# pfnet-research/superpixel-align

Hardware: AMD Instinct MI355X
Metric: images/sec superpixel-align labelling (1024x2048) (higher is better)
Workload: dtype f32 as 2 x f16 planes, f32 accumulate

## Files before the change

### superpixel-align_amd/csrc/spa_common.h

```cpp
#pragma once
#include <hip/hip_runtime.h>
#include <stdint.h>
#include <stdio.h>
#include <string.h>

#include "../../include/spalign.h"

#define SPA_WAVE 64

void spa_set_error(const char *fmt, ...);

#define SPA_HIP(call)                                                                  \
    do {                                                                               \
        hipError_t e_ = (call);                                                        \
        if (e_ != hipSuccess) {                                                        \
            spa_set_error("%s failed: %s (%s:%d)", #call, hipGetErrorString(e_),      \
                          __FILE__, __LINE__);                                         \
            return SPA_ERR_HIP;                                                        \
        }                                                                              \
    } while (0)

#define SPA_ARG(cond)                                                                  \
    do {                                                                               \
        if (!(cond)) {                                                                 \
// ... 61 lines not shown
};

enum {
    PROF_RGB2LAB = 0, PROF_SLIC_ASSIGN, PROF_SLIC_UPDATE, PROF_CONNECT, PROF_STATS,
    PROF_CELL_WEIGHTS, PROF_POOL_MEAN, PROF_POOL_ANCHOR, PROF_KMEANS, PROF_PAINT,
    PROF_DRN_STEM, PROF_DRN_BIAS_ACT, PROF_DRN_CONV, PROF_DRN_CONV32, PROF_DRN_GEMM32, PROF_DRN_GEMM32_N, PROF_WINO_IN, PROF_WINO_OUT, PROF_DRN_GEMM16, PROF_DRN_GEMM16_N, PROF_DRN_CONV16, PROF_DRN_CONV16_128, PROF_DRN_CONV16_256, PROF_DRN_CONV16_1X1, PROF_DRN_CONV16_FRONT, PROF_DRN_CONV_LIGHT, PROF_SLOTS
};

struct spa_ctx {
    int device;
    int n_cu;
    uint32_t *d_status;
    unsigned status_takes;
    void *ws[WS_COUNT];
    size_t ws_bytes[WS_COUNT];
    int prof_on;
    hipEvent_t *prof_ev[PROF_SLOTS];
    int prof_cap[PROF_SLOTS], prof_used[PROF_SLOTS];
    hipStream_t aux[2];
    hipEvent_t ev_fork, ev_join[2];
    int aux_ready;
    int km_attr_done[2];
    int conn_attr_done;
    int conn_claim_ready;
    size_t conn_claim_bytes;
    int upd_wg_per_cu, upd_wg_per_cu8;
    int slic_force_general;
    int zero_line_ready, conv_attr_done, conv32_attr_done, fz_attr_done, gemm16_attr_done, gemm16s_attr_done, nprng_attr_done;
    int rng_seeded;
    int ws_generation;
    int dbg_slic_ldsx;
    int convp_on;
    int convs2_on;
    int convs2_attr_done;
    int rs_key[4], rs_ks[2];
};

#ifdef __HIPCC__
__device__ __forceinline__ unsigned spa_split16_pair(float x0, float x1, float sc, unsigned &l)
{
    unsigned h, lo;
    asm("v_fma_mixlo_f16 %0, %2, %4, 0 op_sel_hi:[0,0,0]\n\t"
        "v_fma_mixhi_f16 %0, %3, %4, 0 op_sel_hi:[0,0,0]\n\t"
        "v_fma_mixlo_f16 %1, %2, %4, -%0 op_sel_hi:[0,0,1]\n\t"
        "v_fma_mixhi_f16 %1, %3, %4, -%0 op_sel:[0,0,1] op_sel_hi:[0,0,1]"
        : "=&v"(h), "=&v"(lo) : "v"(x0), "v"(x1), "v"(sc));
    l = lo;
    return h;
}
#endif

int spa_aux_streams(spa_ctx *ctx);

void spa_prof_mark(spa_ctx *ctx, int slot, int end, hipStream_t s);
struct SpaProfScope {
    spa_ctx *c; int slot; hipStream_t s;
    SpaProfScope(spa_ctx *c_, int slot_, hipStream_t s_) : c(c_), slot(slot_), s(s_) { if (c->prof_on && slot >= 0) spa_prof_mark(c, slot, 0, s); }
    ~SpaProfScope() { if (c->prof_on && slot >= 0) spa_prof_mark(c, slot, 1, s); }
};

int spa_ws_reserve(spa_ctx *ctx, int which, size_t bytes, void **out);
void spa_zero_word(void *word, hipStream_t s);

static inline hipStream_t spa_stream(void *s) { return (hipStream_t)s; }

__device__ __forceinline__ double spa_det_log_pos(double x)
{
    unsigned long long b = (unsigned long long)__double_as_longlong(x);
    int e = (int)((b >> 52) & 0x7ff) - 1023;
    b = (b & 0x000fffffffffffffULL) | 0x3ff0000000000000ULL;
    double m = __longlong_as_double((long long)b);
    if (m > 1.4142135623730951) { m = m * 0.5; e += 1; }
    double s = (m - 1.0) / (m + 1.0);
    double z = s * s;
    double p = 1.0 / 25.0;
    p = p * z + 1.0 / 23.0;
    p = p * z + 1.0 / 21.0;
    p = p * z + 1.0 / 19.0;
    p = p * z + 1.0 / 17.0;
    p = p * z + 1.0 / 15.0;
    p = p * z + 1.0 / 13.0;
    p = p * z + 1.0 / 11.0;
    p = p * z + 1.0 / 9.0;
    p = p * z + 1.0 / 7.0;
    p = p * z + 1.0 / 5.0;
    p = p * z + 1.0 / 3.0;
    p = p * z + 1.0;
    double lnm = 2.0 * s * p;
    double ed = (double)e;
    return ed * 6.93147180369123816490e-01 + (ed * 1.90821492927058770002e-10 + lnm);
}

__device__ __forceinline__ double spa_det_exp(double t)
{
    double kf = floor(t * 1.44269504088896338700e+00 + 0.5);
// ... 27 lines not shown
```

### superpixel-align_amd/csrc/spa_ctx.hip

```cpp
#include <math.h>
#include <stdarg.h>
#include <stdlib.h>

#include "spa_common.h"

static thread_local char g_err[512] = "";

void spa_set_error(const char *fmt, ...)
{
    va_list ap;
    va_start(ap, fmt);
    vsnprintf(g_err, sizeof(g_err), fmt, ap);
    va_end(ap);
}

extern "C" const char *spa_last_error(void) { return g_err; }
extern "C" int spa_version(void) { return 100; }

extern "C" int spa_ctx_create(int device, spa_ctx **out)
{
    SPA_ARG(out != nullptr);
    int n = 0;
    if (hipGetDeviceCount(&n) != hipSuccess || n <= 0) {
        spa_set_error("no HIP device visible: libspalign has no CPU fallback");
        return SPA_ERR_NOGPU;
    }
    if (device < 0) SPA_HIP(hipGetDevice(&device));
    SPA_ARG(device < n);
    SPA_HIP(hipSetDevice(device));
    hipDeviceProp_t prop;
    SPA_HIP(hipGetDeviceProperties(&prop, device));
    if (strncmp(prop.gcnArchName, "gfx950", 6) != 0) {
        spa_set_error("device %d is %s; libspalign is built for gfx950 (MI355X) only", device,
                      prop.gcnArchName);
        return SPA_ERR_NOGPU;
    }
    spa_ctx *ctx = (spa_ctx *)calloc(1, sizeof(spa_ctx));
    ctx->device = device;
    ctx->n_cu = prop.multiProcessorCount;
    if (const char *e = getenv("SPA_SLIC_GENERAL")) ctx->slic_force_general = atoi(e) != 0;
    ctx->convp_on = getenv("SPA_CONVP") ? atoi(getenv("SPA_CONVP")) != 0 : 1;
    ctx->convs2_on = 1;
    SPA_HIP(hipMalloc((void **)&ctx->d_status, 32 * sizeof(uint32_t)));
    SPA_HIP(hipMemset(ctx->d_status, 0, 32 * sizeof(uint32_t)));
    *out = ctx;
    return SPA_OK;
}

extern "C" void spa_ctx_destroy(spa_ctx *ctx)
{
    if (!ctx) return;
    for (int i = 0; i < PROF_SLOTS; ++i) {
        for (int j = 0; j < ctx->prof_cap[i]; ++j) (void)hipEventDestroy(ctx->prof_ev[i][j]);
        free(ctx->prof_ev[i]);
    }
    for (int i = 0; i < WS_COUNT; ++i)
        if (ctx->ws[i]) (void)hipFree(ctx->ws[i]);
    if (ctx->d_status) (void)hipFree(ctx->d_status);
    if (ctx->aux_ready) {
        for (int i = 0; i < 2; ++i) { (void)hipStreamDestroy(ctx->aux[i]); (void)hipEventDestroy(ctx->ev_join[i]); }
        (void)hipEventDestroy(ctx->ev_fork);
    }
    free(ctx);
}

__global__ void k_zero_word(unsigned *w) { *w = 0u; }
void spa_zero_word(void *word, hipStream_t s) { hipLaunchKernelGGL(k_zero_word, dim3(1), dim3(1), 0, s, (unsigned *)word); }

int spa_ws_reserve(spa_ctx *ctx, int which, size_t bytes, void **out)
{
    if (bytes == 0) bytes = 16;
    if (ctx->ws_bytes[which] < bytes) {
        SPA_HIP(hipDeviceSynchronize());
        if (ctx->ws[which]) SPA_HIP(hipFree(ctx->ws[which]));
        ctx->ws[which] = nullptr;
// ... 204 lines not shown
        float4 d;
        if (mode == 1) { d.x = ((const volatile float *)q)[0]; d.y = ((const volatile float *)q)[1]; d.z = ((const volatile float *)q)[2]; d.w = ((const volatile float *)q)[3]; }
        else d = *(const float4 *)q;
        const float ty = (float)(e0.x & 31u) - fy;
        const float dy = (jj & 3) == 3 ? INFINITY : ty * ty;
        const dbg_f32x2 p0 = (dbg_f32x2{dy, dy} + dbg_f32x2{d.x, d.y}) * dbg_f32x2{0.37f, 0.37f} + acc0 * dbg_f32x2{0.001f, 0.001f};
        const dbg_f32x2 p1 = (dbg_f32x2{dy, dy} + dbg_f32x2{d.z, d.w}) * dbg_f32x2{0.37f, 0.37f} + acc1 * dbg_f32x2{0.001f, 0.001f};
        const float dd[4] = {p0.x, p0.y, p1.x, p1.y};
#pragma unroll
        for (int i = 0; i < 4; ++i) {
            const bool take = best[i] > dd[i];
            best[i] = take ? dd[i] : best[i];
            bl[i] = take ? jj : bl[i];
        }
        if (p0.x < 1e30f) acc0 = p0;
        if (p1.x < 1e30f) acc1 = p1;
    }
    float4 r = make_float4(best[0] + (float)bl[0], best[1] + (float)bl[1], best[2] + (float)bl[2], best[3] + (float)bl[3]);
    *(float4 *)(out + ((long long)blockIdx.x * 256 + tid) * 4) = r;
}

extern "C" int spa_debug_lds_probe(spa_ctx *ctx, float *out, int32_t n_wg, int32_t steps, int32_t mode, void *stream)
{
    SPA_ARG(ctx && out && n_wg > 0 && steps > 0 && steps <= 32 && mode >= 0 && mode <= 2);
    hipLaunchKernelGGL(k_debug_lds_probe, dim3((unsigned)n_wg), dim3(256), 0, spa_stream(stream), out, steps, mode, 0.731f);
    SPA_LAUNCH_CHECK();
    return SPA_OK;
}

extern "C" int spa_ws_generation(spa_ctx *ctx) { return ctx ? ctx->ws_generation : -1; }

extern "C" int spa_debug_set(spa_ctx *ctx, int32_t key, int32_t value)
{
    SPA_ARG(ctx && (key == 1 || key == 2 || key == 3) && (value == 0 || value == 1));
    if (key == 1) ctx->convp_on = value;
    else if (key == 3) ctx->convs2_on = value;
    else {
#ifdef SPA_DIAG
        ctx->dbg_slic_ldsx = value;
#else
        SPA_ARG(!"spa_debug_set key 2 (the reproducer variant of k_slic_assign) exists in diagnostic builds only: make EXTRA=-DSPA_DIAG");
#endif
    }
    return SPA_OK;
}

extern "C" int spa_debug_peek(spa_ctx *ctx, int which, size_t offset, size_t bytes, void *host)
{
    if (which == -1) which = WS_DEBUG;
    SPA_ARG(ctx && host && which >= 0 && which < WS_COUNT && offset + bytes <= ctx->ws_bytes[which]);
    SPA_HIP(hipDeviceSynchronize());
    SPA_HIP(hipMemcpy(host, (const char *)ctx->ws[which] + offset, bytes, hipMemcpyDeviceToHost));
    return SPA_OK;
}
```

### superpixel-align_amd/csrc/spa_drn.hip

```cpp
#include "spa_common.h"

__device__ __forceinline__ float bf16_to_f32(unsigned short h) { return __uint_as_float(((unsigned)h) << 16); }
__device__ __forceinline__ unsigned short f32_to_bf16(float f)
{
    unsigned u = __float_as_uint(f);
    if ((u & 0x7fffffffu) > 0x7f800000u) return (unsigned short)((u >> 16) | 0x0040u);
    return (unsigned short)((u + 0x7fffu + ((u >> 16) & 1u)) >> 16);
}

__global__ __launch_bounds__(256) void k_drn_normalise(const float *__restrict__ x, void *__restrict__ out,
                                                       long long npix, int out_bf16, double m0, double m1,
                                                       double m2, double s0, double s1, double s2)
{
    const int b = blockIdx.y;
    const float *src = x + (long long)b * 3 * npix;
    const double mean[3] = {m0, m1, m2}, sd[3] = {s0, s1, s2};
    for (long long p = (long long)blockIdx.x * 256 + threadIdx.x; p < npix; p += (long long)gridDim.x * 256) {
        float v[3];
#pragma unroll
        for (int c = 0; c < 3; ++c) {
            float t = src[c * npix + p] / 255.0f;
            t = (float)((double)t - mean[c]);
            t = (float)((double)t / sd[c]);
            v[c] = t;
        }
        const long long o = ((long long)b * npix + p) * 3;
        if (out_bf16) {
            unsigned short *d = (unsigned short *)out + o;
            d[0] = f32_to_bf16(v[0]); d[1] = f32_to_bf16(v[1]); d[2] = f32_to_bf16(v[2]);
        } else {
            float *d = (float *)out + o;
            d[0] = v[0]; d[1] = v[1]; d[2] = v[2];
        }
    }
}

extern "C" int spa_drn_normalise(spa_ctx *ctx, const float *x, int32_t B, int32_t H, int32_t W, void *out,
                                 int32_t out_dtype, const double *mean3_host, const double *std3_host,
                                 void *stream)
{
    SPA_ARG(ctx && x && out && mean3_host && std3_host && B > 0 && H > 0 && W > 0);
    SPA_ARG(out_dtype == 0 || out_dtype == 1);
    const long long npix = (long long)H * W;
    int gx = (int)((npix + 255) / 256);
    if (gx > 2048) gx = 2048;
    hipLaunchKernelGGL(k_drn_normalise, dim3(gx, B), dim3(256), 0, spa_stream(stream), x, out, npix, out_dtype,
                       mean3_host[0], mean3_host[1], mean3_host[2], std3_host[0], std3_host[1], std3_host[2]);
    SPA_LAUNCH_CHECK();
    return SPA_OK;
}

template <bool POW2>
__global__ __launch_bounds__(256) void k_bias_act_f32(float *__restrict__ y, const float *__restrict__ bias,
                                                      const float *__restrict__ res, unsigned n4, unsigned c4,
                                                      int relu, unsigned *__restrict__ amax = nullptr)
{
    const unsigned stride = gridDim.x * 256u;
    unsigned mx = 0u;
    const float4 *b4 = (const float4 *)bias;
    auto bidx = [&](unsigned i) -> unsigned { return POW2 ? (i & (c4 - 1u)) : (i % c4); };
    auto apply = [&](float4 v, const float4 bb, const float4 r) -> float4 {
        v.x = v.x + bb.x; v.y = v.y + bb.y; v.z = v.z + bb.z; v.w = v.w + bb.w;
        if (res) { v.x = v.x + r.x; v.y = v.y + r.y; v.z = v.z + r.z; v.w = v.w + r.w; }
        if (relu) { v.x = fmaxf(v.x, 0.0f); v.y = fmaxf(v.y, 0.0f); v.z = fmaxf(v.z, 0.0f); v.w = fmaxf(v.w, 0.0f); }
        if (amax)
            mx = max(max(mx, __float_as_uint(v.x) & 0x7fffffffu), max(__float_as_uint(v.y) & 0x7fffffffu,
                     max(__float_as_uint(v.z) & 0x7fffffffu, __float_as_uint(v.w) & 0x7fffffffu)));
        return v;
    };
    unsigned i = blockIdx.x * 256u + threadIdx.x;
    const float4 zero = make_float4(0.0f, 0.0f, 0.0f, 0.0f);
    for (; (unsigned long long)i + 3ull * stride < n4; i += 4u * stride) {
        float4 v[4], r[4];
#pragma unroll
        for (int u = 0; u < 4; ++u) v[u] = ((const float4 *)y)[i + u * stride];
#pragma unroll
        for (int u = 0; u < 4; ++u) r[u] = res ? ((const float4 *)res)[i + u * stride] : zero;
#pragma unroll
        for (int u = 0; u < 4; ++u) ((float4 *)y)[i + u * stride] = apply(v[u], b4[bidx(i + u * stride)], r[u]);
    }
// ... 90 lines not shown
```

### superpixel-align_amd/csrc/spa_stem.hip

```cpp
#include "spa_common.h"

#define ST_TH 16
#define ST_TW 32
#define ST_IH (ST_TH + 8)
#define ST_IW (ST_TW + 8)
#define ST_IPLANE (ST_IH * ST_IW + 8)
#define ST_LH (ST_TH + 2)
#define ST_LW (ST_TW + 2)
#define ST_LP (ST_LH * ST_LW)
#define ST_PS 17
#define ST_K0 148
#define ST_S0 (ST_K0 / 4)
#define ST_S1 (144 / 4)
#define ST_PF 8

typedef float stem_f4 __attribute__((ext_vector_type(4)));

__device__ __forceinline__ unsigned short stem_bf16(float f)
{
    const unsigned u = __float_as_uint(f);
    if ((u & 0x7fffffffu) > 0x7f800000u) return (unsigned short)((u >> 16) | 0x0040u);
    return (unsigned short)((u + 0x7fffu + ((u >> 16) & 1u)) >> 16);
}

// ... 292 lines not shown
            stem_f4 acc = {0.0f, 0.0f, 0.0f, 0.0f};
            const unsigned short *lb = l0_s + (row * ST_LW + col) * SB_L0_PITCH;
#pragma unroll
            for (int s = 0; s < 5; ++s) {
                const stem_bf8 f = *(const stem_bf8 *)(lb + l1off[s]);
                acc = __builtin_amdgcn_mfma_f32_16x16x32_bf16(wa1[s], f, acc, 0, 0, 0);
            }
            const int gy = ty0 + row, gx = tx0 + col;
            if (gy < H && gx < W) {
                uint2 o;
                o.x = (unsigned)stem_bf16_rn(fmaxf(acc[0] + bias1.x, 0.0f)) | ((unsigned)stem_bf16_rn(fmaxf(acc[1] + bias1.y, 0.0f)) << 16);
                o.y = (unsigned)stem_bf16_rn(fmaxf(acc[2] + bias1.z, 0.0f)) | ((unsigned)stem_bf16_rn(fmaxf(acc[3] + bias1.w, 0.0f)) << 16);
                *(uint2 *)(yh + ((((long long)b * H + gy) * W + gx) * 16 + 4 * g)) = o;
            }
        }
        stem_lds_barrier();
    }
}

typedef _Float16 stem_h8 __attribute__((ext_vector_type(8)));
#define SH_PW 48
#define SH_PLANE (ST_IH * SH_PW + 16)
#define SH_COPY (3 * SH_PLANE + 48)
#define SH_L0_PITCH 32
#define SH_IN_S0 4096.0f

__device__ __forceinline__ unsigned short stem_f16_bits(float f)
{
    const _Float16 h = (_Float16)f;
    return __builtin_bit_cast(unsigned short, h);
}
__device__ __forceinline__ float stem_f16_val(unsigned short b) { return (float)__builtin_bit_cast(_Float16, b); }

__global__ __launch_bounds__(256, 2) void k_drn_stem_d_f16x3(const float *__restrict__ xn, int B, int H, int W,
                                                             const unsigned short *__restrict__ wp,
                                                             const float *__restrict__ b0, const float *__restrict__ b1,
                                                             float *__restrict__ y, unsigned *__restrict__ amax_out,
                                                             float *__restrict__ y0)
{
    __shared__ __attribute__((aligned(16))) unsigned short in_h[2][SH_COPY], in_l[2][SH_COPY];
    unsigned amx = 0;
    __shared__ __attribute__((aligned(16))) unsigned short l0_s[ST_LP * SH_L0_PITCH + 64];
    const int tid = threadIdx.x, lane = tid & 63, wv = tid >> 6;
    const int m = lane & 15, g = lane >> 4;
    const long long npix = (long long)H * W;
    const int tiles_x = (W + ST_TW - 1) / ST_TW, tiles_y = (H + ST_TH - 1) / ST_TH;
    const int n_tiles = tiles_x * tiles_y * B;

    stem_h8 w0h[6], w0l[6], w1h[5], w1l[5];
#pragma unroll
    for (int s = 0; s < 6; ++s) {
        w0h[s] = *(const stem_h8 *)(wp + ((size_t)s * 64 + lane) * 8);
        w0l[s] = *(const stem_h8 *)(wp + ((size_t)(6 + s) * 64 + lane) * 8);
    }
#pragma unroll
    for (int s = 0; s < 5; ++s) {
        w1h[s] = *(const stem_h8 *)(wp + ((size_t)(12 + s) * 64 + lane) * 8);
        w1l[s] = *(const stem_h8 *)(wp + ((size_t)(17 + s) * 64 + lane) * 8);
    }
    const float *sc = (const float *)(wp + (size_t)22 * 64 * 8);
    const float unscale0 = sc[0], s1 = sc[1], unscale1 = sc[2];
    const float4 bias0 = *(const float4 *)(b0 + 4 * g), bias1 = *(const float4 *)(b1 + 4 * g);
    int goff[6];
#pragma unroll
    for (int s = 0; s < 6; ++s) {
        const int grp = 4 * s + g;
        const int ky = grp / 3, c = grp - ky * 3;
        goff[s] = grp < 21 ? c * SH_PLANE + ky * SH_PW : 0;
    }
    int l1off[5];
#pragma unroll
    for (int s = 0; s < 5; ++s) {
        int tap = 2 * s + (g >> 1);
        if (tap > 8) tap = 8;
        const int ky = tap / 3, kx = tap - ky * 3;
        l1off[s] = ky * ST_LW + kx;
    }
    constexpr int NE = 3 * ST_IH * ST_IW, NU = (NE + 255) / 256;
    float raw[NU];
    int eiy[NU], eix[NU], elds[NU];
#pragma unroll
    for (int u = 0; u < NU; ++u) {
        int e = tid + u * 256;
        const bool ok = e < NE;
        if (!ok) e = NE - 1;
        const int pix = e / 3, c = e - pix * 3;
        eiy[u] = pix / ST_IW; eix[u] = pix - eiy[u] * ST_IW;
        elds[u] = ok ? c * SH_PLANE + eiy[u] * SH_PW + eix[u] : -1;
        eix[u] = eix[u] * 4 + c;
    }
    auto patch_load = [&](int tile) {
        const int b = tile / (tiles_x * tiles_y), tr = tile - b * (tiles_x * tiles_y);
        const int ty0 = (tr / tiles_x) * ST_TH, tx0 = (tr % tiles_x) * ST_TW;
        const float *src = xn + (long long)b * npix * 3;
#pragma unroll
        for (int u = 0; u < NU; ++u) {
            const int gy = ty0 - 4 + eiy[u], gx = tx0 - 4 + (eix[u] >> 2);
            const int cy = min(max(gy, 0), H - 1), cx = min(max(gx, 0), W - 1);
            raw[u] = src[(unsigned)((cy * W + cx) * 3 + (eix[u] & 3))];
        }
    };
    for (int i = tid; i < SH_COPY; i += 256) { in_h[0][i] = 0; in_h[1][i] = 0; in_l[0][i] = 0; in_l[1][i] = 0; }
    if ((int)blockIdx.x < n_tiles) patch_load(blockIdx.x);
    __syncthreads();

    for (int tile = blockIdx.x; tile < n_tiles; tile += gridDim.x) {
        const int b = tile / (tiles_x * tiles_y), tr = tile - b * (tiles_x * tiles_y);
        const int ty0 = (tr / tiles_x) * ST_TH, tx0 = (tr % tiles_x) * ST_TW;
#pragma unroll
        for (int u = 0; u < NU; ++u) {
            const int ix = eix[u] >> 2;
            const int gy = ty0 - 4 + eiy[u], gx = tx0 - 4 + ix;
            const bool in = (unsigned)gy < (unsigned)H && (unsigned)gx < (unsigned)W;
            if (elds[u] >= 0) {
                const float v = in ? raw[u] * SH_IN_S0 : 0.0f;
                const unsigned short vh = stem_f16_bits(v);
                const unsigned short vl = stem_f16_bits(v - stem_f16_val(vh));
                in_h[0][elds[u]] = vh; in_l[0][elds[u]] = vl;
                if (ix >= 1) { in_h[1][elds[u] - 1] = vh; in_l[1][elds[u] - 1] = vl; }
            }
        }
        stem_lds_barrier();

        for (int t = wv; t < (ST_LP + 15) / 16; t += 4) {
            int p = t * 16 + m;
            if (p > ST_LP - 1) p = ST_LP - 1;
            const int py = p / ST_LW, px = p - py * ST_LW;
            const int boff = py * SH_PW + (px & ~1);
            const unsigned short *bh = in_h[px & 1] + boff, *bl = in_l[px & 1] + boff;
            stem_f4 acc = {0.0f, 0.0f, 0.0f, 0.0f};
#pragma unroll
            for (int s = 0; s < 6; ++s) {
                const uint32_t *qh = (const uint32_t *)(bh + goff[s]), *ql = (const uint32_t *)(bl + goff[s]);
                union { uint32_t u[4]; stem_h8 v; } fh, fl;
                fh.u[0] = qh[0]; fh.u[1] = qh[1]; fh.u[2] = qh[2]; fh.u[3] = qh[3];
                fl.u[0] = ql[0]; fl.u[1] = ql[1]; fl.u[2] = ql[2]; fl.u[3] = ql[3];
                acc = __builtin_amdgcn_mfma_f32_16x16x32_f16(w0l[s], fh.v, acc, 0, 0, 0);
                acc = __builtin_amdgcn_mfma_f32_16x16x32_f16(w0h[s], fl.v, acc, 0, 0, 0);
                acc = __builtin_amdgcn_mfma_f32_16x16x32_f16(w0h[s], fh.v, acc, 0, 0, 0);
            }
            const int q0 = t * 16 + m;
            if (q0 < ST_LP) {
                const int gy = ty0 - 1 + py, gx = tx0 - 1 + px;
                const bool in = gy >= 0 && gy < H && gx >= 0 && gx < W;
                float v[4] = {acc[0] * unscale0 + bias0.x, acc[1] * unscale0 + bias0.y, acc[2] * unscale0 + bias0.z, acc[3] * unscale0 + bias0.w};
                unsigned short vh[4], vl[4];
#pragma unroll
                for (int j = 0; j < 4; ++j) {
                    const float r = in ? fmaxf(v[j], 0.0f) * s1 : 0.0f;
                    vh[j] = stem_f16_bits(r);
                    vl[j] = stem_f16_bits(r - stem_f16_val(vh[j]));
                }
                if (y0 && in && py >= 1 && py <= ST_TH && px >= 1 && px <= ST_TW)
                    *(float4 *)(y0 + ((((long long)b * H + gy) * W + gx) * 16 + 4 * g)) =
                        make_float4(fmaxf(v[0], 0.0f), fmaxf(v[1], 0.0f), fmaxf(v[2], 0.0f), fmaxf(v[3], 0.0f));
                const int sw = (q0 << 2) & 16;
                unsigned short *o = l0_s + q0 * SH_L0_PITCH + 4 * g;
                *(uint2 *)(o + sw) = make_uint2((unsigned)vh[0] | ((unsigned)vh[1] << 16), (unsigned)vh[2] | ((unsigned)vh[3] << 16));
                *(uint2 *)(o + 16 - sw) = make_uint2((unsigned)vl[0] | ((unsigned)vl[1] << 16), (unsigned)vl[2] | ((unsigned)vl[3] << 16));
            }
        }
        stem_lds_barrier();
        if (tile + (int)gridDim.x < n_tiles) patch_load(tile + (int)gridDim.x);

        for (int t = wv; t < 32; t += 4) {
            const int row = t >> 1, col = (t & 1) * 16 + m;
            stem_f4 acc = {0.0f, 0.0f, 0.0f, 0.0f};
            const int qb = row * ST_LW + col;
#pragma unroll
            for (int s = 0; s < 5; ++s) {
                const int q = qb + l1off[s];
                const int sw = (q << 2) & 16;
                const unsigned short *lb = l0_s + q * SH_L0_PITCH + 8 * (g & 1);
                const stem_h8 fh = *(const stem_h8 *)(lb + sw);
                const stem_h8 fl = *(const stem_h8 *)(lb + 16 - sw);
                acc = __builtin_amdgcn_mfma_f32_16x16x32_f16(w1l[s], fh, acc, 0, 0, 0);
                acc = __builtin_amdgcn_mfma_f32_16x16x32_f16(w1h[s], fl, acc, 0, 0, 0);
                acc = __builtin_amdgcn_mfma_f32_16x16x32_f16(w1h[s], fh, acc, 0, 0, 0);
            }
            const int gy = ty0 + row, gx = tx0 + col;
            if (gy < H && gx < W) {
                const float4 o = make_float4(fmaxf(acc[0] * unscale1 + bias1.x, 0.0f), fmaxf(acc[1] * unscale1 + bias1.y, 0.0f),
                                             fmaxf(acc[2] * unscale1 + bias1.z, 0.0f), fmaxf(acc[3] * unscale1 + bias1.w, 0.0f));
                *(float4 *)(y + ((((long long)b * H + gy) * W + gx) * 16 + 4 * g)) = o;
                amx = max(amx, max(max(__float_as_uint(o.x), __float_as_uint(o.y)), max(__float_as_uint(o.z), __float_as_uint(o.w))));
            }
        }
        stem_lds_barrier();
    }
    if (amax_out) {
        for (int o = 32; o > 0; o >>= 1) amx = max(amx, (unsigned)__shfl_xor((int)amx, o));
        if (lane == 0 && amx > *(volatile unsigned *)amax_out) atomicMax(amax_out, amx);
    }
}

#define L2_TH 4
#define L2_TW 32
#define L2_PH (2 * L2_TH + 1)
#define L2_PW (2 * L2_TW + 1)
#define L2_PITCH 40

__global__ __launch_bounds__(256, 2) void k_drn_layer2_f16x3(const float *__restrict__ x, int B, int H, int W, int Ho, int Wo,
                                                             const unsigned short *__restrict__ wp, const float *__restrict__ bias,
                                                             float inv_t, const unsigned *__restrict__ amax_in,
                                                             unsigned *__restrict__ amax_out, float *__restrict__ y)
{
    __shared__ __attribute__((aligned(16))) unsigned short patch[L2_PH * L2_PW * L2_PITCH + 64];
    const int tid = threadIdx.x, lane = tid & 63, wv = tid >> 6;
    const int m = lane & 15, g = lane >> 4;
    const int tiles_x = (Wo + L2_TW - 1) / L2_TW, tiles_y = (Ho + L2_TH - 1) / L2_TH;
    const int n_tiles = tiles_x * tiles_y * B;
    stem_h8 wh[2][5], wl[2][5];
#pragma unroll
    for (int ct = 0; ct < 2; ++ct)
#pragma unroll
        for (int s = 0; s < 5; ++s) {
            wh[ct][s] = *(const stem_h8 *)(wp + ((size_t)((ct * 2 + 0) * 5 + s) * 64 + lane) * 8);
            wl[ct][s] = *(const stem_h8 *)(wp + ((size_t)((ct * 2 + 1) * 5 + s) * 64 + lane) * 8);
        }
    float sc, unscale;
    {
        const unsigned bits = *amax_in;
// ... 267 lines not shown
}

static int stem_impl(spa_ctx *ctx, const float *x, int32_t B, int32_t H, int32_t W,
                     const float *w0, const float *b0, const float *w1, const float *b1,
                     const double *mean3_host, const double *std3_host, void *y, int32_t out_dtype,
                     float *xn_scratch, void *amax_out, void *stream, float *y0)
{
    SPA_ARG(ctx && x && w0 && b0 && w1 && b1 && mean3_host && std3_host && y && B > 0 && H > 0 && W > 0);
    SPA_ARG(!y0 || out_dtype == 2 || out_dtype == 1);
    SPA_ARG(out_dtype == 0 || out_dtype == 1 || out_dtype == 2);
    SpaProfScope prof_(ctx, PROF_DRN_STEM, spa_stream(stream));
    int rc = SPA_OK;
    const long long n_tiles = (long long)((W + ST_TW - 1) / ST_TW) * ((H + ST_TH - 1) / ST_TH) * B;
    SPA_ARG(n_tiles < (1ll << 31));
    SPA_ARG((long long)H * W * 12 < (1ll << 32));
    long long grid = 3ll * ctx->n_cu;
    if (grid > n_tiles) grid = n_tiles;
    if (out_dtype == 1) {
        unsigned short *wp;
        if ((rc = spa_ws_reserve(ctx, WS_STEM_WPACK, (size_t)11 * 64 * 8 * 2, (void **)&wp)) != SPA_OK) return rc;
        hipLaunchKernelGGL(k_stem_pack_bf16, dim3(11), dim3(64), 0, spa_stream(stream), w0, w1, wp);
        unsigned short *xb = (unsigned short *)xn_scratch;
        if (!xb && (rc = spa_ws_reserve(ctx, WS_STEM_IN, (size_t)B * H * W * 3 * sizeof(float), (void **)&xb)) != SPA_OK) return rc;
        if ((rc = spa_drn_normalise(ctx, x, B, H, W, xb, 1, mean3_host, std3_host, stream)) != SPA_OK) return rc;
        hipLaunchKernelGGL(k_drn_stem_d_bf16, dim3((unsigned)grid), dim3(256), 0, spa_stream(stream), (const unsigned short *)xb, B,
                           H, W, (const unsigned short *)wp, b0, (const unsigned short *)(wp + 6 * 64 * 8), b1,
                           (unsigned short *)y, (unsigned short *)y0);
        SPA_LAUNCH_CHECK();
        return SPA_OK;
    }
    float *xn = xn_scratch;
    if (!xn) rc = spa_ws_reserve(ctx, WS_STEM_IN, (size_t)B * H * W * 3 * sizeof(float), (void **)&xn);
    if (rc != SPA_OK) return rc;
    rc = spa_drn_normalise(ctx, x, B, H, W, xn, 0, mean3_host, std3_host, stream);
    if (rc != SPA_OK) return rc;
    if (out_dtype == 2) {
        if (amax_out) spa_zero_word(amax_out, spa_stream(stream));
        unsigned short *wp;
        if ((rc = spa_ws_reserve(ctx, WS_STEM_WPACK, (size_t)22 * 64 * 8 * 2 + 16, (void **)&wp)) != SPA_OK) return rc;
        hipLaunchKernelGGL(k_stem_pack_f16, dim3(23), dim3(64), 0, spa_stream(stream), w0, b0, w1, wp);
        long long g2 = 2ll * ctx->n_cu;
        if (g2 > n_tiles) g2 = n_tiles;
        hipLaunchKernelGGL(k_drn_stem_d_f16x3, dim3((unsigned)g2), dim3(256), 0, spa_stream(stream), (const float *)xn, B, H, W,
                           (const unsigned short *)wp, b0, b1, (float *)y, (unsigned *)amax_out, y0);
        SPA_LAUNCH_CHECK();
        return SPA_OK;
    }
    hipLaunchKernelGGL(k_drn_stem_d, dim3((unsigned)grid), dim3(256), 0, spa_stream(stream), (const float *)xn, B, H, W,
                       w0, b0, w1, b1, y, (int)out_dtype);
    SPA_LAUNCH_CHECK();
    return SPA_OK;
}
```

Baseline: 424.3.

## Pre-split stem input into packed f16 hi/lo planes and add planar stem kernel

The normalise kernel now writes each pixel as a packed f16 hi/lo pair in planar layout, so the stem no longer splits f32 into two f16 values per tile load. A new stem kernel loads whole uint4 pieces for interior tiles, uses byte permutes to build the shifted hi/lo LDS copies, and keeps the layer-0 activations in LDS. It has specialised fast paths that skip bounds checks on interior tiles, plus optional timestamp instrumentation that is compiled out by default. In exchange it adds more register and LDS pressure and a second code path to maintain.

```diff
diff --git a/superpixel-align_amd/csrc/spa_common.h b/superpixel-align_amd/csrc/spa_common.h
--- a/superpixel-align_amd/csrc/spa_common.h
+++ b/superpixel-align_amd/csrc/spa_common.h
@@ -117,6 +117,7 @@
     int dbg_slic_ldsx;
     int convp_on;
     int convs2_on;
+    int stem_planes_on;
     int convs2_attr_done;
     int rs_key[4], rs_ks[2];
 };
@@ -146,6 +147,8 @@
 
 int spa_ws_reserve(spa_ctx *ctx, int which, size_t bytes, void **out);
 void spa_zero_word(void *word, hipStream_t s);
+int spa_drn_normalise_planes(spa_ctx *ctx, const float *x, int32_t B, int32_t H, int32_t W, void *out,
+                             const double *mean3_host, const double *std3_host, void *stream);
 
 static inline hipStream_t spa_stream(void *s) { return (hipStream_t)s; }
 
diff --git a/superpixel-align_amd/csrc/spa_ctx.hip b/superpixel-align_amd/csrc/spa_ctx.hip
--- a/superpixel-align_amd/csrc/spa_ctx.hip
+++ b/superpixel-align_amd/csrc/spa_ctx.hip
@@ -41,6 +41,7 @@
     if (const char *e = getenv("SPA_SLIC_GENERAL")) ctx->slic_force_general = atoi(e) != 0;
     ctx->convp_on = getenv("SPA_CONVP") ? atoi(getenv("SPA_CONVP")) != 0 : 1;
     ctx->convs2_on = 1;
+    ctx->stem_planes_on = 1;
     SPA_HIP(hipMalloc((void **)&ctx->d_status, 32 * sizeof(uint32_t)));
     SPA_HIP(hipMemset(ctx->d_status, 0, 32 * sizeof(uint32_t)));
     *out = ctx;
@@ -311,9 +312,10 @@
 
 extern "C" int spa_debug_set(spa_ctx *ctx, int32_t key, int32_t value)
 {
-    SPA_ARG(ctx && (key == 1 || key == 2 || key == 3) && (value == 0 || value == 1));
+    SPA_ARG(ctx && (key >= 1 && key <= 4) && (value == 0 || value == 1));
     if (key == 1) ctx->convp_on = value;
     else if (key == 3) ctx->convs2_on = value;
+    else if (key == 4) ctx->stem_planes_on = value;
     else {
 #ifdef SPA_DIAG
         ctx->dbg_slic_ldsx = value;
diff --git a/superpixel-align_amd/csrc/spa_drn.hip b/superpixel-align_amd/csrc/spa_drn.hip
--- a/superpixel-align_amd/csrc/spa_drn.hip
+++ b/superpixel-align_amd/csrc/spa_drn.hip
@@ -46,6 +46,51 @@
     if (gx > 2048) gx = 2048;
     hipLaunchKernelGGL(k_drn_normalise, dim3(gx, B), dim3(256), 0, spa_stream(stream), x, out, npix, out_dtype,
                        mean3_host[0], mean3_host[1], mean3_host[2], std3_host[0], std3_host[1], std3_host[2]);
+    SPA_LAUNCH_CHECK();
+    return SPA_OK;
+}
+
+template <int V>
+__global__ __launch_bounds__(256) void k_drn_normalise_planes(const float *__restrict__ x, unsigned *__restrict__ out, long long npix,
+                                                              double m0, double m1, double m2, double s0, double s1, double s2)
+{
+    const int bc = blockIdx.y, c = bc % 3;
+    const float *src = x + (long long)bc * npix;
+    unsigned *dst = out + (long long)bc * npix;
+    const double mean = c == 0 ? m0 : (c == 1 ? m1 : m2), sd = c == 0 ? s0 : (c == 1 ? s1 : s2);
+    for (long long p = ((long long)blockIdx.x * 256 + threadIdx.x) * V; p < npix; p += (long long)gridDim.x * 256 * V) {
+        float v[V];
+        if (V == 4) { const float4 q = *(const float4 *)(src + p); v[0] = q.x; v[1] = q.y; v[2] = q.z; v[V - 1] = q.w; }
+        else v[0] = src[p];
+        unsigned o[V];
+#pragma unroll
+        for (int j = 0; j < V; ++j) {
+            float t = v[j] / 255.0f;
+            t = (float)((double)t - mean);
+            t = (float)((double)t / sd);
+            t = t * 4096.0f;
+            const _Float16 h = (_Float16)t, l = (_Float16)(t - (float)h);
+            o[j] = (unsigned)__builtin_bit_cast(unsigned short, h) | (unsigned)__builtin_bit_cast(unsigned short, l) << 16;
+        }
+        if (V == 4) *(uint4 *)(dst + p) = make_uint4(o[0], o[1], o[2], o[V - 1]);
+        else dst[p] = o[0];
+    }
+}
+
+int spa_drn_normalise_planes(spa_ctx *ctx, const float *x, int32_t B, int32_t H, int32_t W, void *out,
+                             const double *mean3_host, const double *std3_host, void *stream)
+{
+    SPA_ARG(ctx && x && out && mean3_host && std3_host && B > 0 && 3ll * B <= 65535 && H > 0 && W > 0);
+    const long long npix = (long long)H * W;
+    const bool v4 = (npix & 3) == 0 && (((uintptr_t)x | (uintptr_t)out) & 15) == 0;
+    int gx = (int)((npix / (v4 ? 4 : 1) + 255) / 256);
+    if (gx > 1024) gx = 1024;
+    if (v4)
+        hipLaunchKernelGGL(k_drn_normalise_planes<4>, dim3(gx, 3 * B), dim3(256), 0, spa_stream(stream), x, (unsigned *)out, npix,
+                           mean3_host[0], mean3_host[1], mean3_host[2], std3_host[0], std3_host[1], std3_host[2]);
+    else
+        hipLaunchKernelGGL(k_drn_normalise_planes<1>, dim3(gx, 3 * B), dim3(256), 0, spa_stream(stream), x, (unsigned *)out, npix,
+                           mean3_host[0], mean3_host[1], mean3_host[2], std3_host[0], std3_host[1], std3_host[2]);
     SPA_LAUNCH_CHECK();
     return SPA_OK;
 }
diff --git a/superpixel-align_amd/csrc/spa_stem.hip b/superpixel-align_amd/csrc/spa_stem.hip
--- a/superpixel-align_amd/csrc/spa_stem.hip
+++ b/superpixel-align_amd/csrc/spa_stem.hip
@@ -348,11 +348,30 @@
 }
 __device__ __forceinline__ float stem_f16_val(unsigned short b) { return (float)__builtin_bit_cast(_Float16, b); }
 
+#ifdef SPA_ST_STAMPS
+#define ST_Q0 100
+#define ST_NQ 32
+#define ST_STAMP_PARAM , unsigned *__restrict__ dbg
+#define ST_STAMP_ARG , dbg
+#define ST_STAMP_DECL __shared__ unsigned st_stamps[2][ST_NQ][6]; const bool st_wave = blockIdx.x == 77 && (wv == 0 || wv == 3); int st_q = -1, st_n = 0;
+#define ST_STAMP_TILE() do { st_q = (st_n >= ST_Q0 && st_n < ST_Q0 + ST_NQ) ? st_n - ST_Q0 : -1; ++st_n; } while (0)
+#define ST_STAMP(k) do { if (st_wave && st_q >= 0) { const unsigned long long t_ = __builtin_amdgcn_s_memtime(); if (lane == 0) st_stamps[wv ? 1 : 0][st_q][k] = (unsigned)t_; } } while (0)
+#define ST_STAMP_FLUSH() do { if (st_wave && dbg) { asm volatile("s_waitcnt lgkmcnt(0)" ::: "memory"); \
+        for (int i_ = lane; i_ < ST_NQ * 6; i_ += 64) dbg[(wv ? 1 : 0) * (ST_NQ * 6) + i_] = (&st_stamps[wv ? 1 : 0][0][0])[i_]; } } while (0)
+#else
+#define ST_STAMP_PARAM
+#define ST_STAMP_ARG
+#define ST_STAMP_DECL
+#define ST_STAMP_TILE() do { } while (0)
+#define ST_STAMP(k) do { } while (0)
+#define ST_STAMP_FLUSH() do { } while (0)
+#endif
+
 __global__ __launch_bounds__(256, 2) void k_drn_stem_d_f16x3(const float *__restrict__ xn, int B, int H, int W,
                                                              const unsigned short *__restrict__ wp,
                                                              const float *__restrict__ b0, const float *__restrict__ b1,
                                                              float *__restrict__ y, unsigned *__restrict__ amax_out,
-                                                             float *__restrict__ y0)
+                                                             float *__restrict__ y0 ST_STAMP_PARAM)
 {
     __shared__ __attribute__((aligned(16))) unsigned short in_h[2][SH_COPY], in_l[2][SH_COPY];
     unsigned amx = 0;
@@ -362,6 +381,7 @@
     const long long npix = (long long)H * W;
     const int tiles_x = (W + ST_TW - 1) / ST_TW, tiles_y = (H + ST_TH - 1) / ST_TH;
     const int n_tiles = tiles_x * tiles_y * B;
+    ST_STAMP_DECL
 
     stem_h8 w0h[6], w0l[6], w1h[5], w1l[5];
 #pragma unroll
@@ -423,6 +443,8 @@
     for (int tile = blockIdx.x; tile < n_tiles; tile += gridDim.x) {
         const int b = tile / (tiles_x * tiles_y), tr = tile - b * (tiles_x * tiles_y);
         const int ty0 = (tr / tiles_x) * ST_TH, tx0 = (tr % tiles_x) * ST_TW;
+        ST_STAMP_TILE();
+        ST_STAMP(0);
 #pragma unroll
         for (int u = 0; u < NU; ++u) {
             const int ix = eix[u] >> 2;
@@ -436,7 +458,9 @@
                 if (ix >= 1) { in_h[1][elds[u] - 1] = vh; in_l[1][elds[u] - 1] = vl; }
             }
         }
+        ST_STAMP(1);
         stem_lds_barrier();
+        ST_STAMP(2);
 
         for (int t = wv; t < (ST_LP + 15) / 16; t += 4) {
             int p = t * 16 + m;
@@ -476,8 +500,10 @@
                 *(uint2 *)(o + 16 - sw) = make_uint2((unsigned)vl[0] | ((unsigned)vl[1] << 16), (unsigned)vl[2] | ((unsigned)vl[3] << 16));
             }
         }
+        ST_STAMP(3);
         stem_lds_barrier();
         if (tile + (int)gridDim.x < n_tiles) patch_load(tile + (int)gridDim.x);
+        ST_STAMP(4);
 
         for (int t = wv; t < 32; t += 4) {
             const int row = t >> 1, col = (t & 1) * 16 + m;
@@ -502,8 +528,279 @@
                 amx = max(amx, max(max(__float_as_uint(o.x), __float_as_uint(o.y)), max(__float_as_uint(o.z), __float_as_uint(o.w))));
             }
         }
+        ST_STAMP(5);
         stem_lds_barrier();
     }
+    ST_STAMP_FLUSH();
+    if (amax_out) {
+        for (int o = 32; o > 0; o >>= 1) amx = max(amx, (unsigned)__shfl_xor((int)amx, o));
+        if (lane == 0 && amx > *(volatile unsigned *)amax_out) atomicMax(amax_out, amx);
+    }
+}
+
+typedef _Float16 stem_h2 __attribute__((ext_vector_type(2)));
+typedef float stem_f2 __attribute__((ext_vector_type(2)));
+template <bool V> struct stem_tag { static constexpr bool value = V; };
+
+__device__ __forceinline__ void stem_split4(const float *r, uint2 &hh, uint2 &ll)
+{
+    const stem_h2 h01 = __builtin_convertvector((stem_f2){r[0], r[1]}, stem_h2), h23 = __builtin_convertvector((stem_f2){r[2], r[3]}, stem_h2);
+    const float d0 = r[0] - (float)h01[0], d1 = r[1] - (float)h01[1], d2 = r[2] - (float)h23[0], d3 = r[3] - (float)h23[1];
+    const stem_h2 l01 = __builtin_convertvector((stem_f2){d0, d1}, stem_h2), l23 = __builtin_convertvector((stem_f2){d2, d3}, stem_h2);
+    hh = make_uint2(__builtin_bit_cast(unsigned, h01), __builtin_bit_cast(unsigned, h23));
+    ll = make_uint2(__builtin_bit_cast(unsigned, l01), __builtin_bit_cast(unsigned, l23));
+}
+
+#define SP_FU 3
+#define SP_GU 12
+
+template <bool PIECES>
+__global__ __launch_bounds__(256, 2) void k_drn_stem_d_f16x3p(const unsigned *__restrict__ xp, int B, int H, int W,
+                                                              const unsigned short *__restrict__ wp,
+                                                              const float *__restrict__ b0, const float *__restrict__ b1,
+                                                              float *__restrict__ y, unsigned *__restrict__ amax_out,
+                                                              float *__restrict__ y0 ST_STAMP_PARAM)
+{
+    __shared__ __attribute__((aligned(16))) unsigned short in_s[4][SH_COPY];
+    __shared__ __attribute__((aligned(16))) unsigned short l0_s[ST_LP * SH_L0_PITCH + 64];
+    unsigned amx = 0;
+    const int tid = threadIdx.x, lane = tid & 63, wv = tid >> 6;
+    const int m = lane & 15, g = lane >> 4;
+    const unsigned npix = (unsigned)H * (unsigned)W;
+    const int tiles_x = (W + ST_TW - 1) / ST_TW, tiles_y = (H + ST_TH - 1) / ST_TH;
+    const int n_tiles = tiles_x * tiles_y * B;
+    ST_STAMP_DECL
+
+    stem_h8 w0h[6], w0l[6], w1h[5], w1l[5];
+#pragma unroll
+    for (int s = 0; s < 6; ++s) {
+        w0h[s] = *(const stem_h8 *)(wp + ((size_t)s * 64 + lane) * 8);
+        w0l[s] = *(const stem_h8 *)(wp + ((size_t)(6 + s) * 64 + lane) * 8);
+    }
+#pragma unroll
+    for (int s = 0; s < 5; ++s) {
+        w1h[s] = *(const stem_h8 *)(wp + ((size_t)(12 + s) * 64 + lane) * 8);
+        w1l[s] = *(const stem_h8 *)(wp + ((size_t)(17 + s) * 64 + lane) * 8);
+    }
+    const float *sc = (const float *)(wp + (size_t)22 * 64 * 8);
+    const float unscale0 = sc[0], s1 = sc[1], unscale1 = sc[2];
+    const float4 bias0 = *(const float4 *)(b0 + 4 * g), bias1 = *(const float4 *)(b1 + 4 * g);
+    int goff[6];
+#pragma unroll
+    for (int s = 0; s < 6; ++s) {
+        const int grp = 4 * s + g;
+        const int ky = grp / 3, c = grp - ky * 3;
+        goff[s] = grp < 21 ? c * SH_PLANE + ky * SH_PW : 0;
+    }
+    int boff[10];
+#pragma unroll
+    for (int i = 0; i < 10; ++i) {
+        int p = (wv + 4 * i) * 16 + m;
+        if (p > ST_LP - 1) p = ST_LP - 1;
+        const int py = p / ST_LW, px = p - py * ST_LW;
+        boff[i] = (px & 1) * SH_COPY + py * SH_PW + (px & ~1);
+    }
+    int l1a[5], l1b[5];
+#pragma unroll
+    for (int s = 0; s < 5; ++s) {
+        int tap = 2 * s + (g >> 1);
+        if (tap > 8) tap = 8;
+        const int ky = tap / 3, kx = tap - ky * 3;
+        const int q = ((wv >> 1) + ky) * ST_LW + (wv & 1) * 16 + m + kx;
+        const int sw = (q << 2) & 16;
+        l1a[s] = q * SH_L0_PITCH + 8 * (g & 1) + sw;
+        l1b[s] = q * SH_L0_PITCH + 8 * (g & 1) + 16 - sw;
+    }
+
+    unsigned fch[SP_FU];
+    int fpos[SP_FU], flds[SP_FU];
+    int fnext = 0;
+    unsigned pf[5 * SP_FU];
+#pragma unroll
+    for (int u = 0; u < SP_FU; ++u) {
+        int e = tid + u * 256;
+        const bool ok = e < 3 * ST_IH * 10;
+        if (!ok) e = 3 * ST_IH * 10 - 1;
+        const int c = e / (ST_IH * 10), r = e - c * (ST_IH * 10), iy = r / 10, j = r - iy * 10;
+        fch[u] = (unsigned)c * npix;
+        fpos[u] = iy << 8 | 4 * j;
+        flds[u] = ok ? c * SH_PLANE + iy * SH_PW + 4 * j : -1;
+        if (j < 9) fnext |= 1 << u;
+    }
+    static_assert(SP_GU <= 5 * SP_FU, "the border values share the interior pieces' registers");
+    int tid_o = tid;
+    auto border_pos = [&](int u, int &c, int &iy, int &ix) {
+        int e = tid_o + u * 256;
+        const bool ok = e < 3 * ST_IH * ST_IW;
+        if (!ok) e = 3 * ST_IH * ST_IW - 1;
+        c = e / (ST_IH * ST_IW);
+        const int r = e - c * (ST_IH * ST_IW);
+        iy = r / ST_IW; ix = r - iy * ST_IW;
+        return ok;
+    };
+    auto tile_fast = [&](int ty0, int tx0) {
+        return PIECES && ty0 >= 4 && ty0 + ST_TH + 4 <= H && tx0 >= 4 && tx0 + ST_TW + 4 <= W;
+    };
+    auto patch_load = [&](int tile) {
+        const int b = tile / (tiles_x * tiles_y), tr = tile - b * (tiles_x * tiles_y);
+        const int ty0 = (tr / tiles_x) * ST_TH, tx0 = (tr % tiles_x) * ST_TW;
+        const unsigned *img = xp + (long long)b * 3 * npix;
+        if (PIECES) {
+#pragma unroll
+            for (int u = 0; u < SP_FU; ++u) {
+                const int gy = ty0 - 4 + (fpos[u] >> 8), gx = tx0 - 4 + (fpos[u] & 255);
+                const int cy = min(max(gy, 0), H - 1), cx = min(max(gx, 0), W - 4), cn = min(max(gx + 4, 0), W - 1);
+                const unsigned *q = img + (fch[u] + (unsigned)cy * (unsigned)W);
+                const uint4 w4 = *(const uint4 *)(q + cx);
+                pf[5 * u] = w4.x; pf[5 * u + 1] = w4.y; pf[5 * u + 2] = w4.z; pf[5 * u + 3] = w4.w;
+                pf[5 * u + 4] = q[cn];
+            }
+        } else {
+#pragma unroll
+            for (int u = 0; u < SP_GU; ++u) {
+                int c, iy, ix;
+                border_pos(u, c, iy, ix);
+                const int gy = ty0 - 4 + iy, gx = tx0 - 4 + ix;
+                const int cy = min(max(gy, 0), H - 1), cx = min(max(gx, 0), W - 1);
+                pf[u] = img[(unsigned)c * npix + (unsigned)cy * (unsigned)W + (unsigned)cx];
+            }
+        }
+    };
+    for (int i = tid; i < SH_COPY; i += 256) { in_s[0][i] = 0; in_s[1][i] = 0; in_s[2][i] = 0; in_s[3][i] = 0; }
+    if ((int)blockIdx.x < n_tiles) patch_load(blockIdx.x);
+    __syncthreads();
+    __builtin_amdgcn_s_waitcnt(0x0f70);
+
+    for (int tile = blockIdx.x; tile < n_tiles; tile += gridDim.x) {
+        const int b = tile / (tiles_x * tiles_y), tr = tile - b * (tiles_x * tiles_y);
+        const int ty0 = (tr / tiles_x) * ST_TH, tx0 = (tr % tiles_x) * ST_TW;
+        const bool fast = tile_fast(ty0, tx0);
+        asm volatile("" : "+v"(tid_o));
+        ST_STAMP_TILE();
+        ST_STAMP(0);
+
+        auto layer0 = [&](auto tag) {
+            constexpr bool FAST = decltype(tag)::value && PIECES;
+#pragma unroll
+            for (int i = 0; i < 10; ++i) {
+                const int t = wv + 4 * i;
+                if (i < 9 || t < (ST_LP + 15) / 16) {
+                    int bo = boff[i];
+                    asm volatile("" : "+v"(bo));
+                    const unsigned short *bh = &in_s[0][0] + bo, *bl = bh + 2 * SH_COPY;
+                    stem_f4 acc = {0.0f, 0.0f, 0.0f, 0.0f};
+#pragma unroll
+                    for (int s = 0; s < 6; ++s) {
+                        const uint32_t *qh = (const uint32_t *)(bh + goff[s]), *ql = (const uint32_t *)(bl + goff[s]);
+                        union { uint32_t u[4]; stem_h8 v; } xh, xl;
+                        xh.u[0] = qh[0]; xh.u[1] = qh[1]; xh.u[2] = qh[2]; xh.u[3] = qh[3];
+                        xl.u[0] = ql[0]; xl.u[1] = ql[1]; xl.u[2] = ql[2]; xl.u[3] = ql[3];
+                        acc = __builtin_amdgcn_mfma_f32_16x16x32_f16(w0l[s], xh.v, acc, 0, 0, 0);
+                        acc = __builtin_amdgcn_mfma_f32_16x16x32_f16(w0h[s], xl.v, acc, 0, 0, 0);
+                        acc = __builtin_amdgcn_mfma_f32_16x16x32_f16(w0h[s], xh.v, acc, 0, 0, 0);
+                    }
+                    const int q0 = t * 16 + m;
+                    if (i < 9 || q0 < ST_LP) {
+                        const float v[4] = {acc[0] * unscale0 + bias0.x, acc[1] * unscale0 + bias0.y, acc[2] * unscale0 + bias0.z, acc[3] * unscale0 + bias0.w};
+                        bool in = true;
+                        if (!FAST || y0) {
+                            int qo = q0;
+                            asm volatile("" : "+v"(qo));
+                            const int py = qo / ST_LW, px = qo - py * ST_LW;
+                            const int gy = ty0 - 1 + py, gx = tx0 - 1 + px;
+                            if (!FAST) in = gy >= 0 && gy < H && gx >= 0 && gx < W;
+                            if (y0 && in && py >= 1 && py <= ST_TH && px >= 1 && px <= ST_TW)
+                                *(float4 *)(y0 + ((((long long)b * H + gy) * W + gx) * 16 + 4 * g)) =
+                                    make_float4(fmaxf(v[0], 0.0f), fmaxf(v[1], 0.0f), fmaxf(v[2], 0.0f), fmaxf(v[3], 0.0f));
+                        }
+                        float r[4];
+#pragma unroll
+                        for (int j = 0; j < 4; ++j) r[j] = in ? fmaxf(v[j], 0.0f) * s1 : 0.0f;
+                        uint2 hh, ll;
+                        stem_split4(r, hh, ll);
+                        const int sw = (q0 << 2) & 16;
+                        unsigned short *o = l0_s + q0 * SH_L0_PITCH + 4 * g;
+                        *(uint2 *)(o + sw) = hh;
+                        *(uint2 *)(o + 16 - sw) = ll;
+                    }
+                }
+                __builtin_amdgcn_sched_barrier(0);
+            }
+        };
+        auto layer1 = [&](auto tag) {
+            constexpr bool FAST = decltype(tag)::value && PIECES;
+            float *yt = y + ((((long long)b * H + ty0 + (wv >> 1)) * W + tx0 + (wv & 1) * 16 + m) * 16 + 4 * g);
+#pragma unroll
+            for (int i = 0; i < 8; ++i) {
+                stem_f4 acc = {0.0f, 0.0f, 0.0f, 0.0f};
+#pragma unroll
+                for (int s = 0; s < 5; ++s) {
+                    const unsigned short *lb = l0_s + i * (2 * ST_LW * SH_L0_PITCH);
+                    const stem_h8 xh = *(const stem_h8 *)(lb + (i & 1 ? l1b[s] : l1a[s]));
+                    const stem_h8 xl = *(const stem_h8 *)(lb + (i & 1 ? l1a[s] : l1b[s]));
+                    acc = __builtin_amdgcn_mfma_f32_16x16x32_f16(w1l[s], xh, acc, 0, 0, 0);
+                    acc = __builtin_amdgcn_mfma_f32_16x16x32_f16(w1h[s], xl, acc, 0, 0, 0);
+                    acc = __builtin_amdgcn_mfma_f32_16x16x32_f16(w1h[s], xh, acc, 0, 0, 0);
+                }
+                if (FAST || (ty0 + (wv >> 1) + 2 * i < H && tx0 + (wv & 1) * 16 + m < W)) {
+                    const float4 o = make_float4(fmaxf(acc[0] * unscale1 + bias1.x, 0.0f), fmaxf(acc[1] * unscale1 + bias1.y, 0.0f),
+                                                 fmaxf(acc[2] * unscale1 + bias1.z, 0.0f), fmaxf(acc[3] * unscale1 + bias1.w, 0.0f));
+                    *(float4 *)(yt + (long long)i * 2 * W * 16) = o;
+                    amx = max(amx, max(max(__float_as_uint(o.x), __float_as_uint(o.y)), max(__float_as_uint(o.z), __float_as_uint(o.w))));
+                }
+                __builtin_amdgcn_sched_barrier(0);
+            }
+        };
+
+        if (PIECES) {
+#pragma unroll
+            for (int u = 0; u < SP_FU; ++u)
+                if (flds[u] >= 0) {
+                    unsigned f[4] = {pf[5 * u], pf[5 * u + 1], pf[5 * u + 2], pf[5 * u + 3]};
+                    unsigned nx = (fnext >> u & 1) ? pf[5 * u + 4] : 0u;
+                    if (!fast) {
+                        const int gy = ty0 - 4 + (fpos[u] >> 8), gx = tx0 - 4 + (fpos[u] & 255);
+                        const bool row = (unsigned)gy < (unsigned)H;
+                        const bool in = row && (unsigned)gx < (unsigned)W, inn = row && (unsigned)(gx + 4) < (unsigned)W;
+#pragma unroll
+                        for (int k = 0; k < 4; ++k) f[k] = in ? f[k] : 0u;
+                        nx = inn ? nx : 0u;
+                    }
+                    constexpr unsigned SEL_H = 0x05040100u, SEL_L = 0x07060302u;
+                    *(uint2 *)&in_s[0][flds[u]] = make_uint2(__builtin_amdgcn_perm(f[1], f[0], SEL_H), __builtin_amdgcn_perm(f[3], f[2], SEL_H));
+                    *(uint2 *)&in_s[1][flds[u]] = make_uint2(__builtin_amdgcn_perm(f[2], f[1], SEL_H), __builtin_amdgcn_perm(nx, f[3], SEL_H));
+                    *(uint2 *)&in_s[2][flds[u]] = make_uint2(__builtin_amdgcn_perm(f[1], f[0], SEL_L), __builtin_amdgcn_perm(f[3], f[2], SEL_L));
+                    *(uint2 *)&in_s[3][flds[u]] = make_uint2(__builtin_amdgcn_perm(f[2], f[1], SEL_L), __builtin_amdgcn_perm(nx, f[3], SEL_L));
+                }
+        } else {
+#pragma unroll
+            for (int u = 0; u < SP_GU; ++u) {
+                int c, iy, ix;
+                const bool ok = border_pos(u, c, iy, ix);
+                const int gy = ty0 - 4 + iy, gx = tx0 - 4 + ix;
+                const bool in = (unsigned)gy < (unsigned)H && (unsigned)gx < (unsigned)W;
+                if (ok) {
+                    const int o = c * SH_PLANE + iy * SH_PW + ix;
+                    const unsigned short vh = in ? (unsigned short)pf[u] : (unsigned short)0;
+                    const unsigned short vl = in ? (unsigned short)(pf[u] >> 16) : (unsigned short)0;
+                    in_s[0][o] = vh; in_s[2][o] = vl;
+                    if (ix >= 1) { in_s[1][o - 1] = vh; in_s[3][o - 1] = vl; }
+                }
+            }
+        }
+        ST_STAMP(1);
+        stem_lds_barrier();
+        ST_STAMP(2);
+        if (fast) layer0(stem_tag<true>()); else layer0(stem_tag<false>());
+        ST_STAMP(3);
+        stem_lds_barrier();
+        if (tile + (int)gridDim.x < n_tiles) patch_load(tile + (int)gridDim.x);
+        ST_STAMP(4);
+        if (fast) layer1(stem_tag<true>()); else layer1(stem_tag<false>());
+        ST_STAMP(5);
+        stem_lds_barrier();
+    }
+    ST_STAMP_FLUSH();
     if (amax_out) {
         for (int o = 32; o > 0; o >>= 1) amx = max(amx, (unsigned)__shfl_xor((int)amx, o));
         if (lane == 0 && amx > *(volatile unsigned *)amax_out) atomicMax(amax_out, amx);
@@ -837,7 +1134,8 @@
     float *xn = xn_scratch;
     if (!xn) rc = spa_ws_reserve(ctx, WS_STEM_IN, (size_t)B * H * W * 3 * sizeof(float), (void **)&xn);
     if (rc != SPA_OK) return rc;
-    rc = spa_drn_normalise(ctx, x, B, H, W, xn, 0, mean3_host, std3_host, stream);
+    if (out_dtype == 2 && ctx->stem_planes_on) rc = spa_drn_normalise_planes(ctx, x, B, H, W, xn, mean3_host, std3_host, stream);
+    else rc = spa_drn_normalise(ctx, x, B, H, W, xn, 0, mean3_host, std3_host, stream);
     if (rc != SPA_OK) return rc;
     if (out_dtype == 2) {
         if (amax_out) spa_zero_word(amax_out, spa_stream(stream));
@@ -846,8 +1144,22 @@
         hipLaunchKernelGGL(k_stem_pack_f16, dim3(23), dim3(64), 0, spa_stream(stream), w0, b0, w1, wp);
         long long g2 = 2ll * ctx->n_cu;
         if (g2 > n_tiles) g2 = n_tiles;
+#ifdef SPA_ST_STAMPS
+        unsigned *dbg;
+        if ((rc = spa_ws_reserve(ctx, WS_DEBUG, 4096, (void **)&dbg)) != SPA_OK) return rc;
+#endif
+        if (ctx->stem_planes_on) {
+            if (W % 4 == 0 && ((uintptr_t)xn & 15) == 0)
+                hipLaunchKernelGGL(k_drn_stem_d_f16x3p<true>, dim3((unsigned)g2), dim3(256), 0, spa_stream(stream), (const unsigned *)xn, B, H, W,
+                                   (const unsigned short *)wp, b0, b1, (float *)y, (unsigned *)amax_out, y0 ST_STAMP_ARG);
+            else
+                hipLaunchKernelGGL(k_drn_stem_d_f16x3p<false>, dim3((unsigned)g2), dim3(256), 0, spa_stream(stream), (const unsigned *)xn, B, H, W,
+                                   (const unsigned short *)wp, b0, b1, (float *)y, (unsigned *)amax_out, y0 ST_STAMP_ARG);
+            SPA_LAUNCH_CHECK();
+            return SPA_OK;
+        }
         hipLaunchKernelGGL(k_drn_stem_d_f16x3, dim3((unsigned)g2), dim3(256), 0, spa_stream(stream), (const float *)xn, B, H, W,
-                           (const unsigned short *)wp, b0, b1, (float *)y, (unsigned *)amax_out, y0);
+                           (const unsigned short *)wp, b0, b1, (float *)y, (unsigned *)amax_out, y0 ST_STAMP_ARG);
         SPA_LAUNCH_CHECK();
         return SPA_OK;
     }
```

Result: no change. 426.6 (median of 6 runs) (+0.5%).
